# wayveai/fiery

Measured on NVIDIA H100. Metric: camera->BEV lift frames/sec (6-cam 224x480 -> 200x200), higher is better.
Workload: dtype f32

## Files before the change

fiery_b200/csrc/common.cuh:

```cuda
#pragma once
#include <cuda.h>
#include <cuda_runtime.h>
#include <cuda_fp16.h>
#include <stdint.h>
#include <stdio.h>
#include <stdlib.h>
#include "../../include/fiery_b200.h"

namespace fiery {

int set_error(int code, const char* fmt, ...);

#define FIERY_CUDA_CHECK(expr)                                                                              \
    do {                                                                                                    \
        cudaError_t _e = (expr);                                                                            \
        if (_e != cudaSuccess)                                                                              \
            return ::fiery::set_error(FIERY_E_CUDA, "%s failed: %s (%s:%d)", #expr, cudaGetErrorString(_e), \
                                      __FILE__, __LINE__);                                                  \
    } while (0)

#define FIERY_REQUIRE(cond, ...)                                             \
    do {                                                                     \
        if (!(cond)) return ::fiery::set_error(FIERY_E_INVALID, __VA_ARGS__); \
    } while (0)

__device__ __forceinline__ uint32_t smem_addr(const void* p) {
    return static_cast<uint32_t>(__cvta_generic_to_shared(p));
}

__device__ __forceinline__ void mbar_init(uint64_t* bar, uint32_t count) {
    asm volatile("mbarrier.init.shared::cta.b64 [%0], %1;" ::"r"(smem_addr(bar)), "r"(count) : "memory");
}

__device__ __forceinline__ void fence_mbar_init() {
    asm volatile("fence.mbarrier_init.release.cluster;" ::: "memory");
}

__device__ __forceinline__ void fence_proxy_async() {
    asm volatile("fence.proxy.async.shared::cta;" ::: "memory");
}

__device__ __forceinline__ void mbar_arrive_expect_tx(uint64_t* bar, uint32_t bytes) {
    asm volatile("mbarrier.arrive.expect_tx.shared::cta.b64 _, [%0], %1;" ::"r"(smem_addr(bar)), "r"(bytes)
                 : "memory");
}

__device__ __forceinline__ bool mbar_try_wait(uint64_t* bar, uint32_t parity) {
    uint32_t ok;
    asm volatile(
        "{\n\t.reg .pred p;\n\t"
        "mbarrier.try_wait.parity.shared::cta.b64 p, [%1], %2;\n\t"
        "selp.u32 %0, 1, 0, p;\n\t}"
        : "=r"(ok)
        : "r"(smem_addr(bar)), "r"(parity)
        : "memory");
    return ok != 0;
}

__device__ __forceinline__ void mbar_wait(uint64_t* bar, uint32_t parity) {
    uint32_t spins = 0;
    while (!mbar_try_wait(bar, parity)) {
        if (++spins > (1u << 24)) __trap();
// ... 111 lines not shown
```

fiery_b200/csrc/lift_fwd.cu:

```cuda
#include <atomic>
#include <mutex>

#include "lift_plan.cuh"
#include "warp_sample.cuh"

namespace fiery {

constexpr int FIN_THREADS = 256;
__global__ void __launch_bounds__(FIN_THREADS)
finalize_nchw_kernel(float* __restrict__ accum, unsigned char* __restrict__ flags, float* __restrict__ bev,
                     long long pillars, int blocks_per_frame, int clear_marks) {
    constexpr int C = 64;
    const int frame = blockIdx.x / blocks_per_frame;
    const long long pl = static_cast<long long>(blockIdx.x % blocks_per_frame) * FIN_THREADS + threadIdx.x;
    if (pl >= pillars) return;
    unsigned char* f = flags + static_cast<size_t>(frame) * pillars + pl;
    float4 v[C / 4];
    if (*f) {
        float4* row = reinterpret_cast<float4*>(accum + (static_cast<size_t>(frame) * pillars + pl) * C);
#pragma unroll
        for (int q = 0; q < C / 4; ++q) v[q] = row[q];
#pragma unroll
        for (int q = 0; q < C / 4; ++q) row[q] = make_float4(0.f, 0.f, 0.f, 0.f);
        if (clear_marks) *f = 0;
    } else {
#pragma unroll
        for (int q = 0; q < C / 4; ++q) v[q] = make_float4(0.f, 0.f, 0.f, 0.f);
    }
    float* dst = bev + static_cast<size_t>(frame) * C * pillars + pl;
#pragma unroll
    for (int q = 0; q < C / 4; ++q) {
        dst[static_cast<size_t>(4 * q + 0) * pillars] = v[q].x;
        dst[static_cast<size_t>(4 * q + 1) * pillars] = v[q].y;
        dst[static_cast<size_t>(4 * q + 2) * pillars] = v[q].z;
        dst[static_cast<size_t>(4 * q + 3) * pillars] = v[q].w;
// ... 18 lines not shown
__device__ __forceinline__ uint64_t l2_restore_policy(int last_in_lane) {
    return last_in_lane ? l2_evict_normal() : l2_evict_last();
}

__global__ void __launch_bounds__(FT_THREADS)
finalize_tma_kernel(const __grid_constant__ CUtensorMap bev_map, float* __restrict__ accum, unsigned char* __restrict__ touched,
                    long long pillars, int tiles_per_frame, int frame_out0, int clear_marks, int last_in_lane) {
    constexpr int C = 64;
    __shared__ __align__(128) float s_in[FT_P * C];
    __shared__ __align__(128) float s_out[C * FT_P];
    __shared__ __align__(16) float s_zero[C];
    __shared__ __align__(8) uint64_t bar;
    __shared__ unsigned char s_flag[FT_P];
    const int tid = threadIdx.x;
    const int frame = blockIdx.x / tiles_per_frame;
    const long long p0 = static_cast<long long>(blockIdx.x % tiles_per_frame) * FT_P;
    if (tid == 0) {
        tma_prefetch_desc(&bev_map);
        mbar_init(&bar, FT_P);
        fence_mbar_init();
    }
    if (tid >= FT_THREADS - C) s_zero[tid - (FT_THREADS - C)] = 0.f;
    __syncthreads();
    float* row = nullptr;
    unsigned char* mark = nullptr;
    if (tid < FT_P) {
        const long long p = p0 + tid;
        unsigned char f = 0;
        if (p < pillars) {
            mark = touched + static_cast<size_t>(frame) * pillars + p;
            f = *mark;
        }
        s_flag[tid] = f;
        if (f) {
            row = accum + (static_cast<size_t>(frame) * pillars + p) * C;
            mbar_arrive_expect_tx(&bar, C * 4);
            bulk_load_1d(s_in + tid * C, row, C * 4, &bar, l2_evict_last());
        } else {
            mbar_arrive(&bar);
        }
    }
    __syncthreads();
    mbar_wait(&bar, 0);
    {
        const int lane = tid & 31, w = tid >> 5;
        const int pl = (w & 1) * 32 + lane;
        const int chunk0 = ((w >> 1) & 1) * 8;
        const int i0 = (w >> 2) * 4;
        const bool have = s_flag[pl] != 0;
        const float4* src = reinterpret_cast<const float4*>(s_in + pl * C);
        float* dst = s_out + pl;
        const int l7 = lane & 7;
#pragma unroll
        for (int ii = 0; ii < 4; ++ii) {
            const int chunk = chunk0 + ((i0 + ii) ^ l7);
            float4 v = make_float4(0.f, 0.f, 0.f, 0.f);
            if (have) v = src[chunk];
            float* d = dst + chunk * (4 * FT_P);
            d[0] = v.x; d[FT_P] = v.y; d[2 * FT_P] = v.z; d[3 * FT_P] = v.w;
        }
    }
    fence_proxy_async();
    __syncthreads();
    if (tid == 0) tma_store_3d(&bev_map, s_out, static_cast<int>(p0), 0, frame_out0 + frame, l2_evict_first());
    if (row) {
        bulk_store_1d(row, s_zero, C * 4, l2_restore_policy(last_in_lane));
        if (clear_marks) *mark = 0;
    }
    if (tid == 0 || row) tma_store_commit_and_wait();
}

constexpr int FW_P = 64;
constexpr int FW_THREADS = 256;
__global__ void __launch_bounds__(FW_THREADS)
finalize_warp_kernel(const float* __restrict__ accum, const unsigned char* __restrict__ touched, float* __restrict__ bev,
                     long long pillars, int H, int W, int tiles_per_frame, int frame_out0, const float* __restrict__ theta,
                     const unsigned char* __restrict__ copy_mask) {
    constexpr int C = 64;
    __shared__ float s_out[C][FW_P + 1];
    const int tid = threadIdx.x, lane = tid & 31, warp = tid >> 5;
    const int frame = blockIdx.x / tiles_per_frame;
    const long long p0 = static_cast<long long>(blockIdx.x % tiles_per_frame) * FW_P;
    const int gframe = frame_out0 + frame;
    const float* acc_f = accum + static_cast<size_t>(frame) * pillars * C;
    const unsigned char* tch = touched + static_cast<size_t>(frame) * pillars;
    const int l = lane & 7, q = lane >> 3;
#pragma unroll
    for (int pass = 0; pass < 2; ++pass) {
        const int pxl = pass * 32 + warp * 4 + q;
        const long long pix = p0 + pxl;
        float4 a[4], b[4];
        float w[4];
#pragma unroll
        for (int k = 0; k < 4; ++k) {
            a[k] = make_float4(0.f, 0.f, 0.f, 0.f);
            b[k] = a[k];
            w[k] = 0.f;
        }
        if (pix < pillars) {
            const SamplePos s = make_sample(theta, copy_mask, gframe, static_cast<int>(pix), W, H, 0);
#pragma unroll
            for (int k = 0; k < 4; ++k) {
// ... 13 lines not shown
#undef FIERY_BLEND
        s_out[4 * l + 0][pxl] = ra.x; s_out[4 * l + 1][pxl] = ra.y; s_out[4 * l + 2][pxl] = ra.z; s_out[4 * l + 3][pxl] = ra.w;
        s_out[32 + 4 * l + 0][pxl] = rb.x; s_out[32 + 4 * l + 1][pxl] = rb.y; s_out[32 + 4 * l + 2][pxl] = rb.z; s_out[32 + 4 * l + 3][pxl] = rb.w;
    }
    __syncthreads();
    float* dst = bev + static_cast<size_t>(gframe) * C * pillars + p0;
    const uint64_t once = l2_evict_first();
#pragma unroll
    for (int cc = 0; cc < C / (FW_THREADS / 32); ++cc) {
        const int c = warp * (C / (FW_THREADS / 32)) + cc;
#pragma unroll
        for (int half = 0; half < 2; ++half) {
            const int px = half * 32 + lane;
            if (p0 + px < pillars)
                asm volatile("st.global.L2::cache_hint.f32 [%0], %1, %2;"
                             ::"l"(dst + static_cast<size_t>(c) * pillars + px), "f"(s_out[c][px]), "l"(once) : "memory");
        }
    }
}

__global__ void __launch_bounds__(256)
clear_touched_kernel(float* __restrict__ accum, unsigned char* __restrict__ touched, long long n_pillars, int clear_marks,
                     int last_in_lane) {
    const long long p = static_cast<long long>(blockIdx.x) * blockDim.x + threadIdx.x;
    const int lane = threadIdx.x & 31;
    const unsigned char f = p < n_pillars ? touched[p] : 0;
    unsigned m = __ballot_sync(0xffffffffu, f != 0);
    const long long base = p - lane;
    const uint64_t policy = l2_restore_policy(last_in_lane);
    while (m) {
        const int i = __ffs(m) - 1;
        m &= m - 1;
        asm volatile("st.global.L2::cache_hint.v2.f32 [%0], {%1, %1}, %2;"
                     ::"l"(accum + static_cast<size_t>(base + i) * 64 + 2 * lane), "f"(0.f), "l"(policy) : "memory");
    }
    if (f && clear_marks) touched[p] = 0;
}

__global__ void point_indices_kernel(const LiftParams P, int64_t* __restrict__ idx_out, uint8_t* __restrict__ valid_out,
                                     int32_t* __restrict__ pillar_out, long long n_points_total) {
    const long long gid = static_cast<long long>(blockIdx.x) * blockDim.x + threadIdx.x;
    if (gid >= n_points_total) return;
    const int w = static_cast<int>(gid % P.ww);
    long long r = gid / P.ww;
    const int h = static_cast<int>(r % P.hh); r /= P.hh;
    const int d = static_cast<int>(r % P.D); r /= P.D;
// ... 128 lines not shown
        cudaEventRecord(g_timer->ev[2 * g_timer->n], st);
    }
}
static inline void timer_end(cudaStream_t st) {
    if (g_timer && g_timer->n < g_timer->cap) {
        cudaEventRecord(g_timer->ev[2 * g_timer->n + 1], st);
        ++g_timer->n;
    }
}

struct LayoutPass {
    const float* warp_theta;
    const unsigned char* warp_copy;
    bool tma;
    CUtensorMap bev_map;
};
static int prepare_layout_pass(LayoutPass* L, const LiftParams& P, float* bev_out, const float* warp_theta,
                               const unsigned char* warp_copy) {
    *L = LayoutPass{warp_theta, warp_copy, P.pillars % 4 == 0, {}};
    if (P.bev_layout != FIERY_BEV_NCHW || !L->tma || warp_theta) return FIERY_OK;
    return encode_bev_map(&L->bev_map, bev_out, P.pillars, P.C, P.n_frames, FT_P);
}

static void launch_layout_pass(const LayoutPass& L, const LiftParams& P, float* accum, unsigned char* marks, float* bev_out, int frame0,
                               int n_frames, int clear_marks, int last_in_lane, cudaStream_t st) {
    if (L.warp_theta) {
        const int tpf = static_cast<int>((P.pillars + FW_P - 1) / FW_P);
        finalize_warp_kernel<<<static_cast<unsigned>(tpf) * n_frames, FW_THREADS, 0, st>>>(
            accum, marks, bev_out, P.pillars, P.grid.X, P.grid.Y, tpf, frame0, L.warp_theta, L.warp_copy);
    } else if (L.tma) {
        const int tpf = static_cast<int>((P.pillars + FT_P - 1) / FT_P);
        finalize_tma_kernel<<<static_cast<unsigned>(tpf) * n_frames, FT_THREADS, 0, st>>>(
            L.bev_map, accum, marks, P.pillars, tpf, frame0, clear_marks, last_in_lane);
    } else {
        const int bpf = static_cast<int>((P.pillars + FIN_THREADS - 1) / FIN_THREADS);
        finalize_nchw_kernel<<<static_cast<unsigned>(bpf) * n_frames, FIN_THREADS, 0, st>>>(
            accum, marks, bev_out + static_cast<size_t>(frame0) * P.C * P.pillars, P.pillars, bpf, clear_marks);
    }
}

int launch_lift_forward(const LiftParams& P, const void* head, int head_dtype, float* bev_out, void* scratch, const void* plan,
                        const float* warp_theta, const unsigned char* warp_copy, cudaStream_t stream) {
    const bool nchw = P.bev_layout == FIERY_BEV_NCHW;
    FIERY_REQUIRE(scratch != nullptr || !nchw, "NCHW output needs the zeroed scratch buffer of fiery_lift_scratch_bytes()");
    LiftParams Q = P;
    Q.head_f16 = head_dtype == FIERY_DTYPE_F16 ? head : nullptr;
    const int chunk = lift_chunk_frames(P);
    float* accum = static_cast<float*>(scratch);
    unsigned char* scratch_marks =
        nchw ? reinterpret_cast<unsigned char*>(accum + static_cast<size_t>(scratch_frames(P)) * P.pillars * P.C) : nullptr;
    LayoutPass pass;
    int rc = prepare_layout_pass(&pass, P, bev_out, warp_theta, warp_copy);
    if (rc != FIERY_OK) return rc;
    ChainResources* res = nullptr;
    for (int f0 = 0; f0 < P.n_frames; f0 += chunk) {
        const int nf = (P.n_frames - f0 < chunk) ? P.n_frames - f0 : chunk;
        const LaneLayout lanes = lane_layout(P, nf);
        cudaStream_t chain[MAX_LANES] = {stream};
        if (lanes.lanes > 1) {
            if (!res) {
                rc = chain_resources(&res);
                if (rc != FIERY_OK) return rc;
            }
            for (int l = 1; l < lanes.lanes; ++l) chain[l] = res->side[l - 1];
            FIERY_CUDA_CHECK(cudaEventRecord(res->fork, stream));
        }
        for (int g = 0; g < lanes.groups; ++g) {
            const int s0 = group_start(nf, lanes.groups, g), s1 = group_start(nf, lanes.groups, g + 1);
            const int lane = g % lanes.lanes;
            const bool last_in_lane = g + lanes.lanes >= lanes.groups;
            const size_t slice = static_cast<size_t>(lanes.slice0[lane]);
            cudaStream_t st = chain[lane];
            if (lane > 0 && g < lanes.lanes) FIERY_CUDA_CHECK(cudaStreamWaitEvent(st, res->fork, 0));
            Q.frame0 = f0 + s0;
            Q.n_frames = s1 - s0;
            unsigned char* marks = nullptr;
            if (plan) {
                const PlanView v = plan_view(plan, P.n_frames, P.n_cameras, P.n_wtiles, P.pillars, Q.frame0);
                Q.plan_tiles = v.tiles;
                Q.touched = nullptr;
                marks = const_cast<unsigned char*>(v.touched);
            } else {
                Q.plan_tiles = nullptr;
                marks = nchw ? scratch_marks + slice * P.pillars : nullptr;
                Q.touched = marks;
            }
            Q.accum = nchw ? accum + slice * P.pillars * P.C
                           : bev_out + static_cast<size_t>(Q.frame0) * P.pillars * P.C;
            timer_begin(st, 1);
            rc = launch_forward_cols(Q, head, st);
            timer_end(st);
            if (rc != FIERY_OK) return rc;
            if (nchw) {
                timer_begin(st, 2);
                launch_layout_pass(pass, P, Q.accum, marks, bev_out, Q.frame0, Q.n_frames, plan ? 0 : 1, last_in_lane ? 1 : 0, st);
                if (warp_theta) {
                    const long long n = P.pillars * Q.n_frames;
                    clear_touched_kernel<<<static_cast<unsigned>((n + 255) / 256), 256, 0, st>>>(Q.accum, marks, n, plan ? 0 : 1,
                                                                                                 last_in_lane ? 1 : 0);
                }
                timer_end(st);
                FIERY_CUDA_CHECK(cudaGetLastError());
            }
            if (lane > 0 && last_in_lane) {
                FIERY_CUDA_CHECK(cudaEventRecord(res->done[lane - 1], st));
                FIERY_CUDA_CHECK(cudaStreamWaitEvent(stream, res->done[lane - 1], 0));
            }
        }
    }
    return FIERY_OK;
}

struct DetLayout {
    int frames;
    size_t plan, partials, accum, start, cursor, lists, total;
};
static size_t det_align(size_t b) { return (b + 255) & ~static_cast<size_t>(255); }
static DetLayout det_layout(const LiftParams& P) {
    const size_t tpf = static_cast<size_t>(P.n_cameras) * P.n_wtiles;
    const size_t rows = tpf * det_runs_per_tile(P.hh);
    const bool nchw = P.bev_layout == FIERY_BEV_NCHW;
    const size_t per_frame = tpf * PLAN_TILE_BYTES + P.pillars + rows * 64 * 4 + (nchw ? P.pillars * 64 * 4 : 0) + P.pillars * 8 + rows * 4;
    long long c = static_cast<long long>((1ull << 30) / per_frame);
    const int forced = g_max_chunk_frames.load();
    if (forced > 0 && forced < c) c = forced;
// ... 33 lines not shown
    for (int f0 = 0; f0 < P.n_frames; f0 += W.frames) {
        Q.frame0 = f0;
        Q.n_frames = (P.n_frames - f0 < W.frames) ? P.n_frames - f0 : W.frames;
        const unsigned char* marks;
        if (plan) {
            const PlanView v = plan_view(plan, P.n_frames, P.n_cameras, P.n_wtiles, P.pillars, f0);
            Q.plan_tiles = v.tiles;
            marks = v.touched;
        } else {
            const PlanView v = plan_view(ws + W.plan, Q.n_frames, P.n_cameras, P.n_wtiles, P.pillars, 0);
            FIERY_CUDA_CHECK(cudaMemsetAsync(const_cast<unsigned char*>(v.touched), 0, static_cast<size_t>(Q.n_frames) * P.pillars, stream));
            rc = launch_lift_plan(Q, const_cast<unsigned char*>(v.tiles), const_cast<unsigned char*>(v.touched), 0, stream);
            if (rc != FIERY_OK) return rc;
            Q.plan_tiles = v.tiles;
            marks = v.touched;
        }
        Q.accum = partials;
        rc = launch_forward_cols_det(Q, head, stream);
        if (rc != FIERY_OK) return rc;
        float* out = nchw ? accum : bev_out + static_cast<size_t>(f0) * P.pillars * P.C;
        rc = launch_det_reduce(Q, Q.n_frames, Q.plan_tiles, partials, start, cursor, lists, out, nchw ? 0 : 1, stream);
        if (rc != FIERY_OK) return rc;
        if (!nchw) continue;
        launch_layout_pass(pass, P, accum, const_cast<unsigned char*>(marks), bev_out, f0, Q.n_frames, 0, 1, stream);
        FIERY_CUDA_CHECK(cudaGetLastError());
    }
    return FIERY_OK;
}

int launch_point_indices(const LiftParams& P, int64_t* idx_out, uint8_t* valid_out, int32_t* pillar_out, cudaStream_t stream) {
    const long long total = static_cast<long long>(P.n_frames) * P.n_cameras * P.D * P.hh * P.ww;
    if (total == 0) return FIERY_OK;
    const int threads = 256;
    point_indices_kernel<<<static_cast<unsigned>((total + threads - 1) / threads), threads, 0, stream>>>(
        P, idx_out, valid_out, pillar_out, total);
    FIERY_CUDA_CHECK(cudaGetLastError());
    return FIERY_OK;
}

int launch_compose(int n, const float* K, const float* E, float* combined, float* translation, cudaStream_t stream) {
    if (n == 0) return FIERY_OK;
    compose_calibration_kernel<<<(n + 127) / 128, 128, 0, stream>>>(n, K, E, combined, translation);
    FIERY_CUDA_CHECK(cudaGetLastError());
    return FIERY_OK;
}

}
```

fiery_b200/csrc/lift_fwd_cols.cu:

```cuda
#include <string.h>

#include "lift_plan.cuh"

namespace fiery {

constexpr int COLS_NPAIR = DPAD * WT;
constexpr int COLS_EVS = 33;
constexpr int COLS_PLAN_STAGE = 4096;
constexpr int COLS_RUNS_STAGED = (COLS_PLAN_STAGE - PLAN_OFF_RUNS) / 4;
constexpr int CPL = 2;
constexpr int LPU = 64 / CPL;

struct ColsLayout {
    int hh, C;
    int off_bar, off_plan, off_ev, off_prob, off_ctx, off_pillar, total;
    __host__ __device__ ColsLayout(int hh_, int C_, int n_units) : hh(hh_), C(C_) {
        int o = 0;
        off_bar = o;    o += 16;
        off_plan = o;   o += COLS_PLAN_STAGE;
        off_ev = o;     o += n_units * COLS_EVS * 4;
        o = (o + 127) & ~127;
        off_prob = o;   o += hh * DPAD * WT * 4;
        o = (o + 127) & ~127;
        off_ctx = o;    o += hh * C * WT * 4;
// ... 32 lines not shown
    const int d = pair >> 2, col = pair & 3;
    const int j = (d % DD) * 4 + col;
    unsigned* ev = reinterpret_cast<unsigned*>(smem + L.off_ev) + (d / DD) * COLS_EVS;
    int cur = run(k);
    while (m) {
        const int h = __ffs(m) - 1;
        m &= m - 1;
        const int nxt = run(++k);
        atomicOr(ev + h, (1u << j) | (cur >= 0 ? (1u << (4 * DD + j)) : 0u));
        if constexpr (DET) {
            if (cur >= 0) tab[(h - 1) * COLS_NPAIR] = k - 1;
        } else {
            if (cur >= 0) tab[(h - 1) * COLS_NPAIR] = cur;
        }
        cur = nxt;
    }
    if constexpr (DET) tab[(L.hh - 1) * COLS_NPAIR] = cur >= 0 ? k : -1;
    else tab[(L.hh - 1) * COLS_NPAIR] = cur;
}

constexpr int GEO_OFF_CAM = 0, GEO_OFF_U = 48, GEO_OFF_V = 64, GEO_OFF_D = 192;

template <bool POW2, int NT, int DD>
__device__ __forceinline__ void stage_geometry_cols(const LiftParams& P, const ColsLayout& L, unsigned char* smem, int w0,
                                                    unsigned char* touched) {
    constexpr int NRS = NT / COLS_NPAIR >= 4 ? 4 : (NT / COLS_NPAIR >= 2 ? 2 : 1);
    static_assert(NT >= COLS_NPAIR, "one thread per (depth, column) pair at least");
    const float* s_cam = reinterpret_cast<const float*>(smem + L.off_plan + GEO_OFF_CAM);
    const float* s_u = reinterpret_cast<const float*>(smem + L.off_plan + GEO_OFF_U);
    const float* s_v = reinterpret_cast<const float*>(smem + L.off_plan + GEO_OFF_V);
    const float* s_d = reinterpret_cast<const float*>(smem + L.off_plan + GEO_OFF_D);
    int* s_pillar = reinterpret_cast<int*>(smem + L.off_pillar);
    unsigned* s_ev = reinterpret_cast<unsigned*>(smem + L.off_ev);
    CameraTransform T;
#pragma unroll
    for (int i = 0; i < 9; ++i) T.m[i] = s_cam[i];
#pragma unroll
    for (int i = 0; i < 3; ++i) T.t[i] = s_cam[9 + i];
    const PillarMap<POW2> pillar(P.grid);
    const int hh = L.hh;
    const int pair = threadIdx.x / NRS, rs = threadIdx.x % NRS;
    const bool idle = pair >= COLS_NPAIR;
    const int d = idle ? 0 : pair >> 2, col = pair & 3;
    const int unit = d / DD, j = (d % DD) * 4 + col;
    const bool split = hh >= 2 * NRS;
    const int h_lo = idle ? 0 : (split ? (hh * rs) / NRS : 0);
    const int h_hi = idle ? 0 : (split ? (hh * (rs + 1)) / NRS : (rs == 0 ? hh : 0));
    const bool dead = d >= P.D || w0 + col >= P.ww;

    unsigned* ev = s_ev + unit * COLS_EVS;
    int* tab = s_pillar + (idle ? 0 : pair);
    auto run_ends = [&](int h, int before, int now) {
        atomicOr(ev + h, (1u << j) | (before >= 0 ? (1u << (4 * DD + j)) : 0u));
        if (before >= 0) tab[(h - 1) * COLS_NPAIR] = before;
        if (touched && now >= 0) touched[now] = 1;
    };

    int first = -1, prev = -1;
    if (!dead && h_lo < h_hi) {
        const float depth = s_d[d];
        const ColumnTerms ct = column_terms(T, s_u[col], depth);
        int h = h_lo;
#pragma unroll 2
        for (; h < h_hi; ++h) {
            const int cur = pillar(T, ct, s_v[h], depth);
            if (h == h_lo) first = cur;
            else if (cur != prev) run_ends(h, prev, cur);
            prev = cur;
        }
    }
    const int before = __shfl_up_sync(0xffffffffu, prev, 1);
    if (h_lo < h_hi) {
        if (rs > 0 && split) {
            if (first != before) run_ends(h_lo, before, first);
        } else if (touched && first >= 0) {
            touched[first] = 1;
        }
        if (h_hi == hh) tab[(hh - 1) * COLS_NPAIR] = prev;
    }
}


template <int NT>
__device__ __forceinline__ void issue_half_tile(const LiftParams& P, const ColsLayout& L, unsigned char* smem, int img, int w0) {
    const int hh = L.hh;
    const int n_pp = P.use_depth ? hh * DPAD : 0;
    const int n_cp = hh * 64;
    unsigned char* prob_stage = smem + L.off_prob + hh * DPAD * WT * 2;
    unsigned char* ctx_stage = smem + L.off_ctx + hh * 64 * WT * 2;
    const __half* head = static_cast<const __half*>(P.head_f16);
    const size_t plane = static_cast<size_t>(hh) * P.ww;
    const __half* img_base = head + static_cast<size_t>(img) * P.head_channels * plane + w0;
    const int ctx_ch0 = P.use_depth ? P.D : 0;
    for (int p = threadIdx.x; p < n_pp + n_cp; p += NT) {
        if (p < n_pp) {
            const int row = p / DPAD, d = p - row * DPAD;
            if (d < P.D) cp_async_8(prob_stage + p * 8, img_base + d * plane + static_cast<size_t>(row) * P.ww);
        } else {
            const int q = p - n_pp;
            const int row = q >> 6, r = q & 63;
// ... 35 lines not shown
            const float2 hi = __half22float2(*reinterpret_cast<const __half2*>(&v[i].y));
            float4* dst = reinterpret_cast<float4*>(p < n_pp ? prob_base + p * 16 : ctx_base + (p - n_pp) * 16);
            *dst = make_float4(lo.x, lo.y, hi.x, hi.y);
        }
    }
    __syncthreads();
}

template <bool HINT>
__device__ __forceinline__ void red_channels_if(char* dst, const float (&v)[CPL], unsigned bit, uint64_t policy) {
    if (!HINT)
        asm volatile("{\n\t.reg .pred p;\n\tsetp.ne.u32 p, %3, 0;\n\t@p red.global.add.v2.f32 [%0], {%1, %2};\n\t}"
                     :: "l"(dst), "f"(v[0]), "f"(v[1]), "r"(bit) : "memory");
    else
        asm volatile("{\n\t.reg .pred p;\n\tsetp.ne.u32 p, %3, 0;\n\t@p red.global.add.L2::cache_hint.v2.f32 [%0], {%1, %2}, %4;\n\t}"
                     :: "l"(dst), "f"(v[0]), "f"(v[1]), "r"(bit), "l"(policy) : "memory");
}

__device__ __forceinline__ void st_channels_if(char* dst, const float (&v)[CPL], unsigned bit) {
    asm volatile("{\n\t.reg .pred p;\n\tsetp.ne.u32 p, %3, 0;\n\t@p st.global.v2.f32 [%0], {%1, %2};\n\t}"
                 :: "l"(dst), "f"(v[0]), "f"(v[1]), "r"(bit) : "memory");
}

template <int DD, int SD, int COL, bool HINT, bool DET>
__device__ __forceinline__ void flush_slot(unsigned long long (&acc)[CPL][DD][2], unsigned mw, unsigned own, unsigned flush,
                                           const int* plp, char* out, uint64_t policy) {
    constexpr int j = SD * 4 + COL;
    if (mw & (1u << j)) {
        const unsigned pl = static_cast<unsigned>(plp[j]);
        float v[CPL];
#pragma unroll
        for (int k = 0; k < CPL; ++k) v[k] = __fadd_rn(half_of<COL & 1>(acc[k][SD][COL >> 1]), 0.0f);
        if constexpr (DET) st_channels_if(out + static_cast<size_t>(pl) * (64 * 4), v, flush & (1u << j));
        else red_channels_if<HINT>(out + static_cast<size_t>(pl) * (64 * 4), v, flush & (1u << j), policy);
        const unsigned keep = ((own >> j) & 1u) - 1u;
#pragma unroll
        for (int k = 0; k < CPL; ++k) clear_half<COL & 1>(acc[k][SD][COL >> 1], keep);
    }
}

template <int DD, int SD, bool HINT, bool DET>
__device__ __forceinline__ void flush_depth(unsigned long long (&acc)[CPL][DD][2], unsigned mw, unsigned own, unsigned flush,
                                            const int* plp, char* out, uint64_t policy) {
    if (mw & (0xfu << (4 * SD))) {
        flush_slot<DD, SD, 0, HINT, DET>(acc, mw, own, flush, plp, out, policy); flush_slot<DD, SD, 1, HINT, DET>(acc, mw, own, flush, plp, out, policy);
        flush_slot<DD, SD, 2, HINT, DET>(acc, mw, own, flush, plp, out, policy); flush_slot<DD, SD, 3, HINT, DET>(acc, mw, own, flush, plp, out, policy);
    }
    if constexpr (SD + 1 < DD) flush_depth<DD, SD + 1, HINT, DET>(acc, mw, own, flush, plp, out, policy);
}

template <int DD, bool HALF, bool PLANNED, bool HINTS, bool DET>
__global__ void __launch_bounds__((DPAD / DD) * LPU, 2)
lift_forward_cols_kernel(const __grid_constant__ HeadMapsCols head_maps, const LiftParams P) {
    static_assert(!DET || (PLANNED && !HINTS), "the deterministic tile kernel is planned and unhinted");
    constexpr int NU = DPAD / DD;
    constexpr int NT = NU * LPU;
    constexpr int SLOTS = 4 * DD;
    constexpr int UNR = DD == 3 ? 2 : 1;
    static_assert(DPAD % DD == 0 && SLOTS <= 16, "unsupported unit shape");
    extern __shared__ __align__(128) unsigned char smem[];
    const ColsLayout L(P.hh, P.C, NU);
    const int wtile = blockIdx.x % P.n_wtiles;
    const int img_local = blockIdx.x / P.n_wtiles;
    const int img = P.frame0 * P.n_cameras + img_local;
    const int frame = img_local / P.n_cameras;
    const int w0 = wtile * WT;
    const int tid = threadIdx.x;
    const int hh = L.hh;

    uint64_t* bar = reinterpret_cast<uint64_t*>(smem + L.off_bar);
    const unsigned char* rec = PLANNED ? P.plan_tiles + static_cast<size_t>(blockIdx.x) * PLAN_TILE_BYTES : nullptr;
// ... 28 lines not shown
    }
    if (!PLANNED) {
        float* s_u = reinterpret_cast<float*>(smem + L.off_plan + GEO_OFF_U);
        float* s_v = reinterpret_cast<float*>(smem + L.off_plan + GEO_OFF_V);
        float* s_d = reinterpret_cast<float*>(smem + L.off_plan + GEO_OFF_D);
        if (tid < WT) s_u[tid] = (w0 + tid < P.ww) ? P.fu[w0 + tid] : 0.f;
        if (tid >= 32 && tid < 64) s_v[tid - 32] = P.fv[min(tid - 32, hh - 1)];
        if (tid >= 64 && tid < 64 + DPAD) s_d[tid - 64] = (tid - 64 < P.D) ? P.fd[tid - 64] : 0.f;
        if (tid == NT - 1) {
            CameraTransform T;
            load_camera(P.calib_mode, P.calib_a, P.calib_b, img, T);
            float* s_cam = reinterpret_cast<float*>(smem + L.off_plan + GEO_OFF_CAM);
#pragma unroll
            for (int i = 0; i < 9; ++i) s_cam[i] = T.m[i];
#pragma unroll
            for (int i = 0; i < 3; ++i) s_cam[9 + i] = T.t[i];
        }
    }
    __syncthreads();
    if (PLANNED) {
        if (tid < COLS_NPAIR) mbar_wait(bar + 1, 0);
        expand_plan<NT, DD, DET>(L, smem, rec);
    } else {
        unsigned char* touched = P.touched ? P.touched + static_cast<size_t>(frame) * P.pillars : nullptr;
        if (P.grid.pow2[0] && P.grid.pow2[1]) stage_geometry_cols<true, NT, DD>(P, L, smem, w0, touched);
        else stage_geometry_cols<false, NT, DD>(P, L, smem, w0, touched);
    }
    if (HALF) widen_half_tile<NT>(P, L, smem);
    else mbar_wait(bar, 0);
    softmax_depth<NT>(P, reinterpret_cast<float*>(smem + L.off_prob), hh);
    __syncthreads();

    const int unit = tid / LPU;
    const int cl = tid % LPU;
    const float* pp = reinterpret_cast<const float*>(smem + L.off_prob) + unit * DD * WT;
    const float* cp = reinterpret_cast<const float*>(smem + L.off_ctx) + cl * WT;
    const int* plp = reinterpret_cast<const int*>(smem + L.off_pillar) + unit * SLOTS - COLS_NPAIR;
    char* out;
    if constexpr (DET) out = reinterpret_cast<char*>(P.accum + static_cast<size_t>(blockIdx.x) * det_runs_per_tile(hh) * 64 + cl * CPL);
    else out = reinterpret_cast<char*>(P.accum + static_cast<size_t>(frame) * P.pillars * P.C + cl * CPL);
    const unsigned* evp = reinterpret_cast<const unsigned*>(smem + L.off_ev) + unit * COLS_EVS + 1;
    const uint64_t keep = HINTS ? l2_evict_last() : 0;

    unsigned long long acc[CPL][DD][2];
#pragma unroll
    for (int k = 0; k < CPL; ++k)
#pragma unroll
        for (int dd = 0; dd < DD; ++dd) acc[k][dd][0] = acc[k][dd][1] = 0ull;

    unsigned own = 0, flush = 0, mw = 0;
#pragma unroll UNR
    for (int h = 0; h < hh; ++h, pp += DPAD * WT, cp += 64 * WT, plp += COLS_NPAIR, ++evp) {
        const unsigned ev_next = *evp;
        if (mw) flush_depth<DD, 0, HINTS, DET>(acc, mw, own, flush, plp, out, keep);
        ulonglong2 dv[DD];
#pragma unroll
        for (int dd = 0; dd < DD; ++dd) dv[dd] = *reinterpret_cast<const ulonglong2*>(pp + dd * WT);
#pragma unroll
        for (int k = 0; k < CPL; ++k) {
            const ulonglong2 c = *reinterpret_cast<const ulonglong2*>(cp + k * LPU * WT);
#pragma unroll
            for (int dd = 0; dd < DD; ++dd) {
                ffma2(acc[k][dd][0], dv[dd].x, c.x);
                ffma2(acc[k][dd][1], dv[dd].y, c.y);
            }
        }
        own = ev_next & ((1u << SLOTS) - 1u);
        flush = ev_next >> SLOTS;
        mw = own;
    }
#pragma unroll
    for (int j = 0; j < SLOTS; ++j) {
        const int pl = plp[j];
        float v[CPL];
#pragma unroll
        for (int k = 0; k < CPL; ++k) {
            const unsigned long long a = acc[k][j >> 2][(j & 3) >> 1];
            v[k] = (j & 1) ? half_of<1>(a) : half_of<0>(a);
        }
        if constexpr (DET) st_channels_if(out + static_cast<size_t>(static_cast<unsigned>(pl)) * (64 * 4), v, pl >= 0 ? 1u : 0u);
        else red_channels_if<HINTS>(out + static_cast<size_t>(static_cast<unsigned>(pl)) * (64 * 4), v, pl >= 0 ? 1u : 0u, keep);
    }
}

template <int DD, bool HALF, bool PLANNED, bool HINTS, bool DET>
static int launch_forward_cols_t(const LiftParams& P, const void* head, cudaStream_t stream) {
    constexpr int NU = DPAD / DD, NT = NU * LPU;
    const ColsLayout L(P.hh, P.C, NU);
    auto kernel = lift_forward_cols_kernel<DD, HALF, PLANNED, HINTS, DET>;
    static OncePerDevice once;
    int rc = once.run([kernel]() -> int {
        FIERY_CUDA_CHECK(cudaFuncSetAttribute(kernel, cudaFuncAttributeMaxDynamicSharedMemorySize, 227 * 1024));
        FIERY_CUDA_CHECK(cudaFuncSetAttribute(kernel, cudaFuncAttributePreferredSharedMemoryCarveout, cudaSharedmemCarveoutMaxShared));
        return FIERY_OK;
    });
    if (rc != FIERY_OK) return rc;
    FIERY_REQUIRE(L.total <= 227 * 1024, "tile needs %d bytes of shared memory", L.total);
    HeadMapsCols maps;
    if (HALF) {
        memset(&maps, 0, sizeof(maps));
        FIERY_REQUIRE(P.head_f16 != nullptr && (reinterpret_cast<uintptr_t>(P.head_f16) & 7) == 0,
                      "half-precision head tensor must be 8-byte aligned");
    } else {
        rc = encode_head_maps_cols(&maps, head, P, CPL);
        if (rc != FIERY_OK) return rc;
    }
    const long long n_tiles = static_cast<long long>(P.n_frames) * P.n_cameras * P.n_wtiles;
    kernel<<<static_cast<unsigned>(n_tiles), NT, L.total, stream>>>(maps, P);
    FIERY_CUDA_CHECK(cudaGetLastError());
    return FIERY_OK;
}

template <int DD, bool HALF, bool PLANNED>
static int launch_layout_t(const LiftParams& P, const void* head, cudaStream_t stream) {
    return P.bev_layout == FIERY_BEV_NCHW ? launch_forward_cols_t<DD, HALF, PLANNED, true, false>(P, head, stream)
                                          : launch_forward_cols_t<DD, HALF, PLANNED, false, false>(P, head, stream);
}

int launch_forward_cols_det(const LiftParams& P, const void* head, cudaStream_t stream) {
    FIERY_REQUIRE(P.plan_tiles != nullptr, "the deterministic tile kernel needs a plan");
    return P.head_f16 != nullptr ? launch_forward_cols_t<3, true, true, false, true>(P, head, stream)
                                 : launch_forward_cols_t<3, false, true, false, true>(P, head, stream);
}

int launch_forward_cols(const LiftParams& P, const void* head, cudaStream_t stream) {
    const bool half = P.head_f16 != nullptr;
    if (P.plan_tiles != nullptr)
        return half ? launch_layout_t<3, true, true>(P, head, stream) : launch_layout_t<3, false, true>(P, head, stream);
    int n_sm = 0, dev = 0;
    FIERY_CUDA_CHECK(cudaGetDevice(&dev));
    FIERY_CUDA_CHECK(cudaDeviceGetAttribute(&n_sm, cudaDevAttrMultiProcessorCount, dev));
    const long long n_tiles = static_cast<long long>(P.n_frames) * P.n_cameras * P.n_wtiles;
    const long long rem = n_tiles % (2ll * n_sm);
    if (!(rem > 0 && rem <= n_sm))
        return half ? launch_layout_t<3, true, false>(P, head, stream) : launch_layout_t<3, false, false>(P, head, stream);
    return half ? launch_layout_t<2, true, false>(P, head, stream) : launch_layout_t<2, false, false>(P, head, stream);
}

}
```

fiery_b200/csrc/lift_plan.cuh:

```cuda
#pragma once
#include <atomic>
#include <mutex>

#include "lift_tile.cuh"

namespace fiery {

constexpr int PLAN_PAIRS = DPAD * WT;
constexpr int PLAN_RG = 4;
constexpr int PLAN_ND = 4;
constexpr int PLAN_STREAMS = PLAN_RG * WT * PLAN_ND;
constexpr int PLAN_MAX_ROWS = 32;
constexpr int PLAN_CAP = PLAN_PAIRS * PLAN_MAX_ROWS;
constexpr int PLAN_STREAM_CAP = PLAN_CAP + 2 * PLAN_STREAMS;

constexpr int PLAN_OFF_MASK = 0;
constexpr int PLAN_OFF_OFF = PLAN_OFF_MASK + PLAN_PAIRS * 4;
constexpr int PLAN_OFF_SOFF = PLAN_OFF_OFF + PLAN_PAIRS * 2;
constexpr int PLAN_OFF_COUNTS = PLAN_OFF_SOFF + PLAN_STREAMS * 2;
constexpr int PLAN_OFF_RUNS = PLAN_OFF_COUNTS + 16;
constexpr int PLAN_OFF_STREAMS = PLAN_OFF_RUNS + PLAN_CAP * 4;
constexpr int PLAN_TILE_BYTES = (PLAN_OFF_STREAMS + PLAN_STREAM_CAP * 4 + 127) & ~127;

__host__ __device__ inline int det_runs_per_tile(int rows) { return PLAN_PAIRS * rows; }
// ... 15 lines not shown
    PlanView v;
    v.tiles = base + static_cast<size_t>(frame0) * n_cameras * n_wtiles * PLAN_TILE_BYTES;
    v.touched = base + static_cast<size_t>(n_frames_total) * n_cameras * n_wtiles * PLAN_TILE_BYTES + static_cast<size_t>(frame0) * pillars;
    return v;
}

struct OncePerDevice {
    std::atomic<int> done[64];
    std::mutex mu;
    template <typename F>
    int run(F&& configure) {
        int dev = 0;
        FIERY_CUDA_CHECK(cudaGetDevice(&dev));
        std::atomic<int>& flag = done[dev & 63];
        if (flag.load(std::memory_order_acquire)) return FIERY_OK;
        std::lock_guard<std::mutex> lock(mu);
        if (flag.load(std::memory_order_relaxed)) return FIERY_OK;
        const int rc = configure();
        if (rc == FIERY_OK) flag.store(1, std::memory_order_release);
        return rc;
    }
};

struct LaunchTimer {
    static constexpr int MAX = 64;
    cudaEvent_t ev[2 * MAX];
    int kind[MAX];
    int n = 0, cap = 0;
};

__host__ __device__ __forceinline__ int plan_group_row(int rows, int rg) { return (rows * rg) / PLAN_RG; }

int check_lift_geometry(const LiftParams& P);
int encode_bev_map(CUtensorMap* map, float* bev, long long pillars, int channels, int n_frames, int box_pillars);
int launch_lift_plan(const LiftParams& P, unsigned char* tiles, unsigned char* touched, int want_streams, cudaStream_t stream);
int launch_forward_cols(const LiftParams& P, const void* head, cudaStream_t stream);
int launch_forward_cols_det(const LiftParams& P, const void* head, cudaStream_t stream);
int launch_det_reduce(const LiftParams& P, int nf, const unsigned char* tiles, const float* partials, int* start, int* cursor,
                      int* lists, float* out, int zero_empty, cudaStream_t stream);
int launch_lift_forward(const LiftParams& P, const void* head, int head_dtype, float* bev_out, void* scratch, const void* plan,
                        const float* warp_theta, const unsigned char* warp_copy, cudaStream_t stream);
int launch_lift_forward_det(const LiftParams& P, const void* head, int head_dtype, float* bev_out, void* workspace, const void* plan,
                            const float* warp_theta, const unsigned char* warp_copy, cudaStream_t stream);
size_t lift_scratch_bytes(const LiftParams& P);
size_t lift_det_workspace_bytes(const LiftParams& P);
int lift_forward_launches(const LiftParams& P);
void lift_set_max_chunk_frames(int n);
void lift_set_timer(LaunchTimer* t);
int launch_point_indices(const LiftParams& P, int64_t* idx_out, uint8_t* valid_out, int32_t* pillar_out, cudaStream_t stream);
int launch_compose(int n, const float* K, const float* E, float* combined, float* translation, cudaStream_t stream);
size_t lift_backward_relayout_bytes(const LiftParams& P);
int launch_lift_backward(const LiftParams& P, const void* head, float* workspace, const void* plan, cudaStream_t stream);

}
```

Baseline: 69220.

## Chain lift and layout kernels with programmatic dependent launch; mark touched pillars at flush

Launches the forward column kernel, the finalize/layout kernels and the clear kernel with programmatic stream serialization, and adds griddepcontrol wait/launch_dependents calls so each kernel's prologue (geometry staging, softmax, TMA setup) can overlap the tail of the previous kernel in the same lane. Touched-pillar marking moves from geometry staging to the accumulation flush, so it happens after the dependency wait and does not race with the previous kernel's clear. This is meant to hide launch gaps and prologue latency between back-to-back kernels. PDL is disabled when the launch timer is active, and ordering now relies on the placement of the wait calls.

```diff
diff --git a/fiery_b200/csrc/common.cuh b/fiery_b200/csrc/common.cuh
--- a/fiery_b200/csrc/common.cuh
+++ b/fiery_b200/csrc/common.cuh
@@ -38,6 +38,13 @@
 
 __device__ __forceinline__ void fence_proxy_async() {
     asm volatile("fence.proxy.async.shared::cta;" ::: "memory");
+}
+
+__device__ __forceinline__ void grid_dependency_wait() {
+    asm volatile("griddepcontrol.wait;" ::: "memory");
+}
+__device__ __forceinline__ void allow_dependent_launch() {
+    asm volatile("griddepcontrol.launch_dependents;" ::: "memory");
 }
 
 __device__ __forceinline__ void mbar_arrive_expect_tx(uint64_t* bar, uint32_t bytes) {
diff --git a/fiery_b200/csrc/lift_fwd.cu b/fiery_b200/csrc/lift_fwd.cu
--- a/fiery_b200/csrc/lift_fwd.cu
+++ b/fiery_b200/csrc/lift_fwd.cu
@@ -11,6 +11,8 @@
 finalize_nchw_kernel(float* __restrict__ accum, unsigned char* __restrict__ flags, float* __restrict__ bev,
                      long long pillars, int blocks_per_frame, int clear_marks) {
     constexpr int C = 64;
+    allow_dependent_launch();
+    grid_dependency_wait();
     const int frame = blockIdx.x / blocks_per_frame;
     const long long pl = static_cast<long long>(blockIdx.x % blocks_per_frame) * FIN_THREADS + threadIdx.x;
     if (pl >= pillars) return;
@@ -75,6 +77,7 @@
     }
     if (tid >= FT_THREADS - C) s_zero[tid - (FT_THREADS - C)] = 0.f;
     __syncthreads();
+    grid_dependency_wait();
     float* row = nullptr;
     unsigned char* mark = nullptr;
     if (tid < FT_P) {
@@ -95,6 +98,7 @@
     }
     __syncthreads();
     mbar_wait(&bar, 0);
+    allow_dependent_launch();
     {
         const int lane = tid & 31, w = tid >> 5;
         const int pl = (w & 1) * 32 + lane;
@@ -131,6 +135,8 @@
                      const unsigned char* __restrict__ copy_mask) {
     constexpr int C = 64;
     __shared__ float s_out[C][FW_P + 1];
+    allow_dependent_launch();
+    grid_dependency_wait();
     const int tid = threadIdx.x, lane = tid & 31, warp = tid >> 5;
     const int frame = blockIdx.x / tiles_per_frame;
     const long long p0 = static_cast<long long>(blockIdx.x % tiles_per_frame) * FW_P;
@@ -190,6 +196,8 @@
 __global__ void __launch_bounds__(256)
 clear_touched_kernel(float* __restrict__ accum, unsigned char* __restrict__ touched, long long n_pillars, int clear_marks,
                      int last_in_lane) {
+    allow_dependent_launch();
+    grid_dependency_wait();
     const long long p = static_cast<long long>(blockIdx.x) * blockDim.x + threadIdx.x;
     const int lane = threadIdx.x & 31;
     const unsigned char f = p < n_pillars ? touched[p] : 0;
@@ -364,21 +372,20 @@
     return encode_bev_map(&L->bev_map, bev_out, P.pillars, P.C, P.n_frames, FT_P);
 }
 
-static void launch_layout_pass(const LayoutPass& L, const LiftParams& P, float* accum, unsigned char* marks, float* bev_out, int frame0,
-                               int n_frames, int clear_marks, int last_in_lane, cudaStream_t st) {
+static int launch_layout_pass(const LayoutPass& L, const LiftParams& P, float* accum, unsigned char* marks, float* bev_out, int frame0,
+                              int n_frames, int clear_marks, int last_in_lane, cudaStream_t st, bool chained) {
     if (L.warp_theta) {
         const int tpf = static_cast<int>((P.pillars + FW_P - 1) / FW_P);
-        finalize_warp_kernel<<<static_cast<unsigned>(tpf) * n_frames, FW_THREADS, 0, st>>>(
-            accum, marks, bev_out, P.pillars, P.grid.X, P.grid.Y, tpf, frame0, L.warp_theta, L.warp_copy);
+        return launch_chain_kernel(finalize_warp_kernel, static_cast<unsigned>(tpf) * n_frames, FW_THREADS, 0, st, chained,
+                                   accum, marks, bev_out, P.pillars, P.grid.X, P.grid.Y, tpf, frame0, L.warp_theta, L.warp_copy);
     } else if (L.tma) {
         const int tpf = static_cast<int>((P.pillars + FT_P - 1) / FT_P);
-        finalize_tma_kernel<<<static_cast<unsigned>(tpf) * n_frames, FT_THREADS, 0, st>>>(
-            L.bev_map, accum, marks, P.pillars, tpf, frame0, clear_marks, last_in_lane);
-    } else {
-        const int bpf = static_cast<int>((P.pillars + FIN_THREADS - 1) / FIN_THREADS);
-        finalize_nchw_kernel<<<static_cast<unsigned>(bpf) * n_frames, FIN_THREADS, 0, st>>>(
-            accum, marks, bev_out + static_cast<size_t>(frame0) * P.C * P.pillars, P.pillars, bpf, clear_marks);
-    }
+        return launch_chain_kernel(finalize_tma_kernel, static_cast<unsigned>(tpf) * n_frames, FT_THREADS, 0, st, chained,
+                                   L.bev_map, accum, marks, P.pillars, tpf, frame0, clear_marks, last_in_lane);
+    }
+    const int bpf = static_cast<int>((P.pillars + FIN_THREADS - 1) / FIN_THREADS);
+    return launch_chain_kernel(finalize_nchw_kernel, static_cast<unsigned>(bpf) * n_frames, FIN_THREADS, 0, st, chained,
+                               accum, marks, bev_out + static_cast<size_t>(frame0) * P.C * P.pillars, P.pillars, bpf, clear_marks);
 }
 
 int launch_lift_forward(const LiftParams& P, const void* head, int head_dtype, float* bev_out, void* scratch, const void* plan,
@@ -407,6 +414,7 @@
             for (int l = 1; l < lanes.lanes; ++l) chain[l] = res->side[l - 1];
             FIERY_CUDA_CHECK(cudaEventRecord(res->fork, stream));
         }
+        bool chained[MAX_LANES] = {};
         for (int g = 0; g < lanes.groups; ++g) {
             const int s0 = group_start(nf, lanes.groups, g), s1 = group_start(nf, lanes.groups, g + 1);
             const int lane = g % lanes.lanes;
@@ -429,20 +437,22 @@
             }
             Q.accum = nchw ? accum + slice * P.pillars * P.C
                            : bev_out + static_cast<size_t>(Q.frame0) * P.pillars * P.C;
+            const bool pdl = g_timer == nullptr;
             timer_begin(st, 1);
-            rc = launch_forward_cols(Q, head, st);
+            rc = launch_forward_cols(Q, head, st, chained[lane]);
             timer_end(st);
             if (rc != FIERY_OK) return rc;
+            chained[lane] = pdl;
             if (nchw) {
                 timer_begin(st, 2);
-                launch_layout_pass(pass, P, Q.accum, marks, bev_out, Q.frame0, Q.n_frames, plan ? 0 : 1, last_in_lane ? 1 : 0, st);
-                if (warp_theta) {
+                rc = launch_layout_pass(pass, P, Q.accum, marks, bev_out, Q.frame0, Q.n_frames, plan ? 0 : 1, last_in_lane ? 1 : 0, st, pdl);
+                if (rc == FIERY_OK && warp_theta) {
                     const long long n = P.pillars * Q.n_frames;
-                    clear_touched_kernel<<<static_cast<unsigned>((n + 255) / 256), 256, 0, st>>>(Q.accum, marks, n, plan ? 0 : 1,
-                                                                                                 last_in_lane ? 1 : 0);
+                    rc = launch_chain_kernel(clear_touched_kernel, static_cast<unsigned>((n + 255) / 256), 256, 0, st, pdl, Q.accum, marks,
+                                             n, plan ? 0 : 1, last_in_lane ? 1 : 0);
                 }
                 timer_end(st);
-                FIERY_CUDA_CHECK(cudaGetLastError());
+                if (rc != FIERY_OK) return rc;
             }
             if (lane > 0 && last_in_lane) {
                 FIERY_CUDA_CHECK(cudaEventRecord(res->done[lane - 1], st));
@@ -522,8 +532,8 @@
         rc = launch_det_reduce(Q, Q.n_frames, Q.plan_tiles, partials, start, cursor, lists, out, nchw ? 0 : 1, stream);
         if (rc != FIERY_OK) return rc;
         if (!nchw) continue;
-        launch_layout_pass(pass, P, accum, const_cast<unsigned char*>(marks), bev_out, f0, Q.n_frames, 0, 1, stream);
-        FIERY_CUDA_CHECK(cudaGetLastError());
+        rc = launch_layout_pass(pass, P, accum, const_cast<unsigned char*>(marks), bev_out, f0, Q.n_frames, 0, 1, stream, false);
+        if (rc != FIERY_OK) return rc;
     }
     return FIERY_OK;
 }
diff --git a/fiery_b200/csrc/lift_fwd_cols.cu b/fiery_b200/csrc/lift_fwd_cols.cu
--- a/fiery_b200/csrc/lift_fwd_cols.cu
+++ b/fiery_b200/csrc/lift_fwd_cols.cu
@@ -78,8 +78,7 @@
 constexpr int GEO_OFF_CAM = 0, GEO_OFF_U = 48, GEO_OFF_V = 64, GEO_OFF_D = 192;
 
 template <bool POW2, int NT, int DD>
-__device__ __forceinline__ void stage_geometry_cols(const LiftParams& P, const ColsLayout& L, unsigned char* smem, int w0,
-                                                    unsigned char* touched) {
+__device__ __forceinline__ void stage_geometry_cols(const LiftParams& P, const ColsLayout& L, unsigned char* smem, int w0) {
     constexpr int NRS = NT / COLS_NPAIR >= 4 ? 4 : (NT / COLS_NPAIR >= 2 ? 2 : 1);
     static_assert(NT >= COLS_NPAIR, "one thread per (depth, column) pair at least");
     const float* s_cam = reinterpret_cast<const float*>(smem + L.off_plan + GEO_OFF_CAM);
@@ -106,10 +105,9 @@
 
     unsigned* ev = s_ev + unit * COLS_EVS;
     int* tab = s_pillar + (idle ? 0 : pair);
-    auto run_ends = [&](int h, int before, int now) {
+    auto run_ends = [&](int h, int before) {
         atomicOr(ev + h, (1u << j) | (before >= 0 ? (1u << (4 * DD + j)) : 0u));
         if (before >= 0) tab[(h - 1) * COLS_NPAIR] = before;
-        if (touched && now >= 0) touched[now] = 1;
     };
 
     int first = -1, prev = -1;
@@ -121,17 +119,13 @@
         for (; h < h_hi; ++h) {
             const int cur = pillar(T, ct, s_v[h], depth);
             if (h == h_lo) first = cur;
-            else if (cur != prev) run_ends(h, prev, cur);
+            else if (cur != prev) run_ends(h, prev);
             prev = cur;
         }
     }
     const int before = __shfl_up_sync(0xffffffffu, prev, 1);
     if (h_lo < h_hi) {
-        if (rs > 0 && split) {
-            if (first != before) run_ends(h_lo, before, first);
-        } else if (touched && first >= 0) {
-            touched[first] = 1;
-        }
+        if (rs > 0 && split && first != before) run_ends(h_lo, before);
         if (h_hi == hh) tab[(hh - 1) * COLS_NPAIR] = prev;
     }
 }
@@ -213,9 +207,13 @@
                  :: "l"(dst), "f"(v[0]), "f"(v[1]), "r"(bit) : "memory");
 }
 
-template <int DD, int SD, int COL, bool HINT, bool DET>
+__device__ __forceinline__ void mark_pillar(const LiftParams& P, const char* out, unsigned pl) {
+    P.touched[static_cast<size_t>(out - reinterpret_cast<const char*>(P.accum)) / (64 * 4) + pl] = 1;
+}
+
+template <int DD, int SD, int COL, bool HINT, bool DET, bool MARK>
 __device__ __forceinline__ void flush_slot(unsigned long long (&acc)[CPL][DD][2], unsigned mw, unsigned own, unsigned flush,
-                                           const int* plp, char* out, uint64_t policy) {
+                                           const int* plp, char* out, const LiftParams& P, uint64_t policy) {
     constexpr int j = SD * 4 + COL;
     if (mw & (1u << j)) {
         const unsigned pl = static_cast<unsigned>(plp[j]);
@@ -224,20 +222,23 @@
         for (int k = 0; k < CPL; ++k) v[k] = __fadd_rn(half_of<COL & 1>(acc[k][SD][COL >> 1]), 0.0f);
         if constexpr (DET) st_channels_if(out + static_cast<size_t>(pl) * (64 * 4), v, flush & (1u << j));
         else red_channels_if<HINT>(out + static_cast<size_t>(pl) * (64 * 4), v, flush & (1u << j), policy);
+        if constexpr (MARK) if (flush & (1u << j)) mark_pillar(P, out, pl);
         const unsigned keep = ((own >> j) & 1u) - 1u;
 #pragma unroll
         for (int k = 0; k < CPL; ++k) clear_half<COL & 1>(acc[k][SD][COL >> 1], keep);
     }
 }
 
-template <int DD, int SD, bool HINT, bool DET>
+template <int DD, int SD, bool HINT, bool DET, bool MARK>
 __device__ __forceinline__ void flush_depth(unsigned long long (&acc)[CPL][DD][2], unsigned mw, unsigned own, unsigned flush,
-                                            const int* plp, char* out, uint64_t policy) {
+                                            const int* plp, char* out, const LiftParams& P, uint64_t policy) {
     if (mw & (0xfu << (4 * SD))) {
-        flush_slot<DD, SD, 0, HINT, DET>(acc, mw, own, flush, plp, out, policy); flush_slot<DD, SD, 1, HINT, DET>(acc, mw, own, flush, plp, out, policy);
-        flush_slot<DD, SD, 2, HINT, DET>(acc, mw, own, flush, plp, out, policy); flush_slot<DD, SD, 3, HINT, DET>(acc, mw, own, flush, plp, out, policy);
-    }
-    if constexpr (SD + 1 < DD) flush_depth<DD, SD + 1, HINT, DET>(acc, mw, own, flush, plp, out, policy);
+        flush_slot<DD, SD, 0, HINT, DET, MARK>(acc, mw, own, flush, plp, out, P, policy);
+        flush_slot<DD, SD, 1, HINT, DET, MARK>(acc, mw, own, flush, plp, out, P, policy);
+        flush_slot<DD, SD, 2, HINT, DET, MARK>(acc, mw, own, flush, plp, out, P, policy);
+        flush_slot<DD, SD, 3, HINT, DET, MARK>(acc, mw, own, flush, plp, out, P, policy);
+    }
+    if constexpr (SD + 1 < DD) flush_depth<DD, SD + 1, HINT, DET, MARK>(acc, mw, own, flush, plp, out, P, policy);
 }
 
 template <int DD, bool HALF, bool PLANNED, bool HINTS, bool DET>
@@ -312,14 +313,14 @@
         if (tid < COLS_NPAIR) mbar_wait(bar + 1, 0);
         expand_plan<NT, DD, DET>(L, smem, rec);
     } else {
-        unsigned char* touched = P.touched ? P.touched + static_cast<size_t>(frame) * P.pillars : nullptr;
-        if (P.grid.pow2[0] && P.grid.pow2[1]) stage_geometry_cols<true, NT, DD>(P, L, smem, w0, touched);
-        else stage_geometry_cols<false, NT, DD>(P, L, smem, w0, touched);
+        if (P.grid.pow2[0] && P.grid.pow2[1]) stage_geometry_cols<true, NT, DD>(P, L, smem, w0);
+        else stage_geometry_cols<false, NT, DD>(P, L, smem, w0);
     }
     if (HALF) widen_half_tile<NT>(P, L, smem);
     else mbar_wait(bar, 0);
     softmax_depth<NT>(P, reinterpret_cast<float*>(smem + L.off_prob), hh);
     __syncthreads();
+    if constexpr (!DET) grid_dependency_wait();
 
     const int unit = tid / LPU;
     const int cl = tid % LPU;
@@ -331,6 +332,7 @@
     else out = reinterpret_cast<char*>(P.accum + static_cast<size_t>(frame) * P.pillars * P.C + cl * CPL);
     const unsigned* evp = reinterpret_cast<const unsigned*>(smem + L.off_ev) + unit * COLS_EVS + 1;
     const uint64_t keep = HINTS ? l2_evict_last() : 0;
+    constexpr bool MARK = HINTS && !PLANNED;
 
     unsigned long long acc[CPL][DD][2];
 #pragma unroll
@@ -342,7 +344,7 @@
 #pragma unroll UNR
     for (int h = 0; h < hh; ++h, pp += DPAD * WT, cp += 64 * WT, plp += COLS_NPAIR, ++evp) {
         const unsigned ev_next = *evp;
-        if (mw) flush_depth<DD, 0, HINTS, DET>(acc, mw, own, flush, plp, out, keep);
+        if (mw) flush_depth<DD, 0, HINTS, DET, MARK>(acc, mw, own, flush, plp, out, P, keep);
         ulonglong2 dv[DD];
 #pragma unroll
         for (int dd = 0; dd < DD; ++dd) dv[dd] = *reinterpret_cast<const ulonglong2*>(pp + dd * WT);
@@ -370,11 +372,12 @@
         }
         if constexpr (DET) st_channels_if(out + static_cast<size_t>(static_cast<unsigned>(pl)) * (64 * 4), v, pl >= 0 ? 1u : 0u);
         else red_channels_if<HINTS>(out + static_cast<size_t>(static_cast<unsigned>(pl)) * (64 * 4), v, pl >= 0 ? 1u : 0u, keep);
+        if constexpr (MARK) if (pl >= 0) mark_pillar(P, out, static_cast<unsigned>(pl));
     }
 }
 
 template <int DD, bool HALF, bool PLANNED, bool HINTS, bool DET>
-static int launch_forward_cols_t(const LiftParams& P, const void* head, cudaStream_t stream) {
+static int launch_forward_cols_t(const LiftParams& P, const void* head, cudaStream_t stream, bool chained) {
     constexpr int NU = DPAD / DD, NT = NU * LPU;
     const ColsLayout L(P.hh, P.C, NU);
     auto kernel = lift_forward_cols_kernel<DD, HALF, PLANNED, HINTS, DET>;
@@ -396,35 +399,33 @@
         if (rc != FIERY_OK) return rc;
     }
     const long long n_tiles = static_cast<long long>(P.n_frames) * P.n_cameras * P.n_wtiles;
-    kernel<<<static_cast<unsigned>(n_tiles), NT, L.total, stream>>>(maps, P);
-    FIERY_CUDA_CHECK(cudaGetLastError());
-    return FIERY_OK;
+    return launch_chain_kernel(kernel, static_cast<unsigned>(n_tiles), NT, L.total, stream, chained, maps, P);
 }
 
 template <int DD, bool HALF, bool PLANNED>
-static int launch_layout_t(const LiftParams& P, const void* head, cudaStream_t stream) {
-    return P.bev_layout == FIERY_BEV_NCHW ? launch_forward_cols_t<DD, HALF, PLANNED, true, false>(P, head, stream)
-                                          : launch_forward_cols_t<DD, HALF, PLANNED, false, false>(P, head, stream);
+static int launch_layout_t(const LiftParams& P, const void* head, cudaStream_t stream, bool chained) {
+    return P.bev_layout == FIERY_BEV_NCHW ? launch_forward_cols_t<DD, HALF, PLANNED, true, false>(P, head, stream, chained)
+                                          : launch_forward_cols_t<DD, HALF, PLANNED, false, false>(P, head, stream, chained);
 }
 
 int launch_forward_cols_det(const LiftParams& P, const void* head, cudaStream_t stream) {
     FIERY_REQUIRE(P.plan_tiles != nullptr, "the deterministic tile kernel needs a plan");
-    return P.head_f16 != nullptr ? launch_forward_cols_t<3, true, true, false, true>(P, head, stream)
-                                 : launch_forward_cols_t<3, false, true, false, true>(P, head, stream);
-}
-
-int launch_forward_cols(const LiftParams& P, const void* head, cudaStream_t stream) {
+    return P.head_f16 != nullptr ? launch_forward_cols_t<3, true, true, false, true>(P, head, stream, false)
+                                 : launch_forward_cols_t<3, false, true, false, true>(P, head, stream, false);
+}
+
+int launch_forward_cols(const LiftParams& P, const void* head, cudaStream_t stream, bool chained) {
     const bool half = P.head_f16 != nullptr;
     if (P.plan_tiles != nullptr)
-        return half ? launch_layout_t<3, true, true>(P, head, stream) : launch_layout_t<3, false, true>(P, head, stream);
+        return half ? launch_layout_t<3, true, true>(P, head, stream, chained) : launch_layout_t<3, false, true>(P, head, stream, chained);
     int n_sm = 0, dev = 0;
     FIERY_CUDA_CHECK(cudaGetDevice(&dev));
     FIERY_CUDA_CHECK(cudaDeviceGetAttribute(&n_sm, cudaDevAttrMultiProcessorCount, dev));
     const long long n_tiles = static_cast<long long>(P.n_frames) * P.n_cameras * P.n_wtiles;
     const long long rem = n_tiles % (2ll * n_sm);
     if (!(rem > 0 && rem <= n_sm))
-        return half ? launch_layout_t<3, true, false>(P, head, stream) : launch_layout_t<3, false, false>(P, head, stream);
-    return half ? launch_layout_t<2, true, false>(P, head, stream) : launch_layout_t<2, false, false>(P, head, stream);
-}
-
-}
+        return half ? launch_layout_t<3, true, false>(P, head, stream, chained) : launch_layout_t<3, false, false>(P, head, stream, chained);
+    return half ? launch_layout_t<2, true, false>(P, head, stream, chained) : launch_layout_t<2, false, false>(P, head, stream, chained);
+}
+
+}
diff --git a/fiery_b200/csrc/lift_plan.cuh b/fiery_b200/csrc/lift_plan.cuh
--- a/fiery_b200/csrc/lift_plan.cuh
+++ b/fiery_b200/csrc/lift_plan.cuh
@@ -61,6 +61,23 @@
     }
 };
 
+template <typename... Params, typename... Args>
+int launch_chain_kernel(void (*kernel)(Params...), unsigned grid, unsigned block, size_t smem, cudaStream_t stream, bool chained,
+                        Args&&... args) {
+    cudaLaunchAttribute attr;
+    attr.id = cudaLaunchAttributeProgrammaticStreamSerialization;
+    attr.val.programmaticStreamSerializationAllowed = 1;
+    cudaLaunchConfig_t cfg = {};
+    cfg.gridDim = dim3(grid);
+    cfg.blockDim = dim3(block);
+    cfg.dynamicSmemBytes = smem;
+    cfg.stream = stream;
+    cfg.attrs = &attr;
+    cfg.numAttrs = chained ? 1 : 0;
+    FIERY_CUDA_CHECK(cudaLaunchKernelEx(&cfg, kernel, std::forward<Args>(args)...));
+    return FIERY_OK;
+}
+
 struct LaunchTimer {
     static constexpr int MAX = 64;
     cudaEvent_t ev[2 * MAX];
@@ -73,7 +90,7 @@
 int check_lift_geometry(const LiftParams& P);
 int encode_bev_map(CUtensorMap* map, float* bev, long long pillars, int channels, int n_frames, int box_pillars);
 int launch_lift_plan(const LiftParams& P, unsigned char* tiles, unsigned char* touched, int want_streams, cudaStream_t stream);
-int launch_forward_cols(const LiftParams& P, const void* head, cudaStream_t stream);
+int launch_forward_cols(const LiftParams& P, const void* head, cudaStream_t stream, bool chained);
 int launch_forward_cols_det(const LiftParams& P, const void* head, cudaStream_t stream);
 int launch_det_reduce(const LiftParams& P, int nf, const unsigned char* tiles, const float* partials, int* start, int* cursor,
                       int* lists, float* out, int zero_empty, cudaStream_t stream);
```

Measured after the change: 69330 (median of 6 runs). Within noise of the previous version (+0.2%).
